# rssalessio/TZDDPC

Measured on AMD Instinct MI355X. Metric: MPC steps/sec (batched trajectories), double-integrator N=20, higher is better.
Workload: dtype f64

## Files before the change

### tzddpc_amd/csrc/tz_ipm.hip.h

```cpp
#pragma once

#define TZ_MINWAVES 4
#define TZ_RLEV_CARRY_MAX 2
#define TZ_RLEV_GATE 1e6
#define TZ_SEED_VIOL_MAX 0.1

struct TzEll { int L, VL; const TzEllEnt* ent; const int* seg; const double* val; const unsigned short* idx; };
#define TZ_ELL_D 8
typedef __attribute__((address_space(1))) const char* tz_gptr;
typedef __attribute__((address_space(1))) const tz_d2* tz_gd2ptr;
#define TZ_ELL_FETCH4(base, r0, r1, r2, r3) \
  tz_d2 r0, r1, r2, r3; \
  { tz_gptr q0 = base, q1 = base + stride, q2 = base + 2 * (size_t)stride, q3 = base + 3 * (size_t)stride; \
    asm volatile("" : "+s"(q0), "+s"(q1), "+s"(q2), "+s"(q3)); \
    r0 = *(tz_gd2ptr)(q0 + lo); r1 = *(tz_gd2ptr)(q1 + lo); r2 = *(tz_gd2ptr)(q2 + lo); r3 = *(tz_gd2ptr)(q3 + lo); \
    base += 4 * (size_t)stride; }
#define TZ_ELL_TERM(r) (r.x * *reinterpret_cast<const double*>(b + tz_ell_off(r.y)))
#define TZ_ELL_APPLY4(a0, a1, r0, r1, r2, r3) { a0 += TZ_ELL_TERM(r0); a1 += TZ_ELL_TERM(r1); a0 += TZ_ELL_TERM(r2); a1 += TZ_ELL_TERM(r3); }
static_assert(TZ_ELL_D == 8, "the windows of tz_ell_walk / tz_ell_walk2 are written out for eight records");
__device__ inline double tz_ell_walk(const char* base_, unsigned lo, int L, unsigned stride, const double* in) {
  double a0 = 0.0, a1 = 0.0;
  const char* b = reinterpret_cast<const char*>(in);
  tz_gptr base = (tz_gptr)base_;
  int e = 0;
// ... 215 lines not shown
  else if (NF == 1) { if (!U0) tz_wave_reduce3<OP0, OP0, OP0, 1>(a, b, c); else if (NV > 1 && !U1) tz_wave_reduce3<OP1, OP1, OP1, 1>(b, a, c); else tz_wave_reduce3<OP2, OP2, OP2, 1>(c, a, b); }
  const int tt = tz_tid();
  int lane = tt & 63, w = tt >> 6;
  double* rb_ = red + (par ? 16 : 0);
  par ^= 1;
  if (lane == 0) {
    rb_[w] = U0 ? __builtin_bit_cast(double, (unsigned long long)ua) : a;
    if (NV > 1) rb_[4 + w] = U1 ? __builtin_bit_cast(double, (unsigned long long)ub) : b;
    if (NV > 2) rb_[8 + w] = U2 ? __builtin_bit_cast(double, (unsigned long long)uc) : c;
  }
  __syncthreads();
  const double ra = tz_fold4<OP0>(rb_), rb = (NV > 1) ? tz_fold4<OP1>(rb_ + 4) : 0.0, rc = (NV > 2) ? tz_fold4<OP2>(rb_ + 8) : 0.0;
  a = ra; if (NV > 1) b = rb; if (NV > 2) c = rc;
}

template <int NCG, int W0 = 0, int NW = TZ_NWAVES>
__device__ inline void tz_gemvT_partial(const double* M, int rows, int nzp, const double* in, double* part) {
  const int tt = tz_tid();
  const int lane = tt & 63, w = (tt >> 6) - W0;
  constexpr int UR = (NCG <= 2) ? 8 : 4;
  double acc[NCG];
#pragma unroll
  for (int g = 0; g < NCG; ++g) acc[g] = 0.0;
  int r = w;
  for (; r + (UR - 1) * NW < rows; r += UR * NW) {
    double v[UR], m[UR][NCG];
#pragma unroll
    for (int u = 0; u < UR; ++u) {
      v[u] = in[r + u * NW];
      const double* row = M + (size_t)(r + u * NW) * nzp;
#pragma unroll
      for (int g = 0; g < NCG; ++g) { const int c = min(lane + 64 * g, nzp - 1); m[u][g] = row[c]; }
    }
#pragma unroll
    for (int u = 0; u < UR; ++u)
#pragma unroll
      for (int g = 0; g < NCG; ++g) acc[g] += m[u][g] * v[u];
  }
  for (; r < rows; r += NW) {
    const double v = in[r];
    const double* row = M + (size_t)r * nzp;
#pragma unroll
    for (int g = 0; g < NCG; ++g) { const int c = min(lane + 64 * g, nzp - 1); acc[g] += row[c] * v; }
  }
#pragma unroll
  for (int g = 0; g < NCG; ++g) { const int c = lane + 64 * g; if (c < nzp) part[w * nzp + c] = acc[g]; }
}
__device__ inline double tz_gemvT_get(const double* part, int nzp, int c) {
  return (part[c] + part[nzp + c]) + (part[2 * nzp + c] + part[3 * nzp + c]);
}
__device__ inline double tz_gemvT_get3(const double* part, int nzp, int c) {
  return (part[c] + part[nzp + c]) + part[2 * nzp + c];
}

template <bool COMPACT>
__device__ inline void tz_ell_gemv_walk(const IpmParams& p, const double* in, double* pl) {
  const int t = tz_tid(), L = p.eg.L;
  int v0 = 0;
  if constexpr (!COMPACT) {
    for (; v0 + TZ_THREADS < p.eg.VL; v0 += 2 * TZ_THREADS) {
      double s0, s1;
      tz_ell_walk2(reinterpret_cast<const char*>(p.eg.ent + (size_t)v0 * L), reinterpret_cast<const char*>(p.eg.ent + (size_t)(v0 + TZ_THREADS) * L),
                   (unsigned)t * 16u, L, TZ_THREADS * 16u, in, s0, s1);
      pl[v0 + t] = s0; pl[v0 + TZ_THREADS + t] = s1;
    }
  }
  for (; v0 < p.eg.VL; v0 += TZ_THREADS) {
    if constexpr (COMPACT) pl[v0 + t] = tz_ell_walk_c(p.eg.val + (size_t)v0 * L + t, p.eg.idx + (size_t)v0 * L + t, L, TZ_THREADS, in);
    else pl[v0 + t] = tz_ell_walk(reinterpret_cast<const char*>(p.eg.ent + (size_t)v0 * L), (unsigned)t * 16u, L, TZ_THREADS * 16u, in);
  }
}
template <int MAXR>
__device__ inline void tz_ell_gemv_sum(const double* pl, const int (&rseg)[MAXR], double (&out)[MAXR]) {
#pragma unroll
  for (int k = 0; k < MAXR; ++k) {
    double a = 0.0;
    int sg = rseg[k];
    asm volatile("" : "+v"(sg));
    const int first = sg & 0xffff, cnt = sg >> 16;
    for (int j = 0; j < cnt; ++j) a += pl[first + j];
    out[k] = a;
  }
}
template <int MAXR, bool COMPACT>
__device__ inline void tz_ell_gemv(const IpmParams& p, const double* in, double* pl, const int (&rseg)[MAXR], double (&out)[MAXR]) {
  __syncthreads();
  tz_ell_gemv_walk<COMPACT>(p, in, pl);
  __syncthreads();
  tz_ell_gemv_sum<MAXR>(pl, rseg, out);
}

template <bool COMPACT>
__device__ inline void tz_ell_gemvT_part(const IpmParams& p, const double* in, double* pl) {
  constexpr int NL = TZ_THREADS - 64;
  const int l = tz_tid() - 64, L = p.et.L;
  for (int v0 = 0; v0 < p.et.VL; v0 += NL) {
    if constexpr (COMPACT) pl[v0 + l] = tz_ell_walk_c(p.et.val + (size_t)v0 * L + l, p.et.idx + (size_t)v0 * L + l, L, NL, in);
    else pl[v0 + l] = tz_ell_walk(reinterpret_cast<const char*>(p.et.ent + (size_t)v0 * L), (unsigned)l * 16u, L, NL * 16u, in);
  }
}
__device__ inline double tz_ell_colsum(const double* pl, int cseg) {
  double a = 0.0;
  asm volatile("" : "+v"(cseg));
  const int first = cseg & 0xffff, cnt = cseg >> 16;
  for (int j = 0; j < cnt; ++j) a += pl[first + j];
  return a;
}

struct TzStage { double a[4]; double b[2]; double w; };

__device__ inline double tz_ld_pinned(const double* p) {
  unsigned long long u = __hip_atomic_load((const unsigned long long*)p, __ATOMIC_RELAXED, __HIP_MEMORY_SCOPE_WAVEFRONT);
  return __builtin_bit_cast(double, u);
}

__device__ inline void tz_form_H(const IpmParams& p, double* Hq, const double* wv, const int* kl) {
  const int lane = threadIdx.x & 63, wave = threadIdx.x >> 6;
  const int k = lane >> 4, blk = (lane >> 2) & 3, ij = lane & 3;
  const int Tz = p.Tz;
  const unsigned rowbytes = (unsigned)(Tz + 1) * 128u;
  const unsigned laneoff = (unsigned)(4 * k + ij) * 8u;
  const char* gp = (const char*)p.Gp;
  const int it0 = __builtin_amdgcn_readfirstlane(p.item_ptr[wave]), it1 = __builtin_amdgcn_readfirstlane(p.item_ptr[wave + 1]);
  for (int it = it0; it < it1; ++it) {
    const IpmItem item = p.items[it];
    const int I0 = __builtin_amdgcn_readfirstlane(item.I0), q0 = __builtin_amdgcn_readfirstlane(item.q0);
    const int nq = __builtin_amdgcn_readfirstlane(item.nq), klen = __builtin_amdgcn_readfirstlane(item.klen);
    const int* kli = kl + __builtin_amdgcn_readfirstlane(item.kptr);
    double acc[4][2];
#pragma unroll
    for (int ii = 0; ii < 4; ++ii) { acc[ii][0] = 0.0; acc[ii][1] = 0.0; }
    unsigned aoff[4], boff[2];
#pragma unroll
    for (int ii = 0; ii < 4; ++ii) aoff[ii] = (unsigned)((I0 + ii < Tz) ? (I0 + ii) : Tz) * 128u + laneoff;
#pragma unroll
    for (int nn = 0; nn < 2; ++nn) { const int J = 4 * (q0 + nn) + blk; boff[nn] = (unsigned)((nn < nq && J < Tz) ? J : Tz) * 128u + laneoff; }
    auto load = [&](int kk, TzStage& st) {
      const int kc = __builtin_amdgcn_readfirstlane(kli[kk]);
      st.w = wv[4 * kc + k];
      const char* prow = gp + (size_t)kc * rowbytes;
#pragma unroll
      for (int ii = 0; ii < 4; ++ii) st.a[ii] = tz_ld_pinned((const double*)(prow + aoff[ii]));
#pragma unroll
      for (int nn = 0; nn < 2; ++nn) st.b[nn] = tz_ld_pinned((const double*)(prow + boff[nn]));
    };
    auto fma8 = [&](const TzStage& st) {
#pragma unroll
      for (int ii = 0; ii < 4; ++ii) {
        const double a = st.a[ii] * st.w;
        acc[ii][0] = __builtin_amdgcn_mfma_f64_4x4x4f64(a, st.b[0], acc[ii][0], 0, 0, 0);
        acc[ii][1] = __builtin_amdgcn_mfma_f64_4x4x4f64(a, st.b[1], acc[ii][1], 0, 0, 0);
      }
    };
    TzStage s0, s1, s2, s3;
    load(0, s0); load(1, s1); load(2, s2);
    for (int kk = 0; kk < klen; kk += 4) {
      load(kk + 3, s3); fma8(s0);
      load(kk + 4, s0); fma8(s1);
      load(kk + 5, s1); fma8(s2);
      load(kk + 6, s2); fma8(s3);
    }
    const int i = lane >> 4, j = lane & 3;
#pragma unroll
    for (int ii = 0; ii < 4; ++ii) {
      const int I = I0 + ii;
      if (I >= Tz) continue;
#pragma unroll
      for (int nn = 0; nn < 2; ++nn) {
        const int q = q0 + nn;
// ... 399 lines not shown
  }
  else for (int i = t; i < p.nklist; i += TZ_THREADS) kl[i] = p.klist[i];
  if (fused) {
    const int n = F0.fin.n, m = F0.fin.m, nv = F0.fin.N * m;
    const int n1 = (F0.tube.pmax + 1) * n * n, n2 = n1 + (F0.tube.pmax > 0 ? F0.tube.pmax : 1) * (n + m) * n;
    for (int i = t; i < n2; i += TZ_THREADS) tbl[i] = (i < n1) ? F0.tube.CKpow[i] : F0.tube.T[i - n1];
    double* ec = tbl + n2;
    const double* plA = F0.plant.A + (size_t)b * F0.plant.A_stride;
    const double* plB = F0.plant.Bm + (size_t)b * F0.plant.B_stride;
    for (int i = t; i < n * n; i += TZ_THREADS) { ec[i] = plA[i]; ec[2 * n * m + n * n + n + i] = F0.fin.R2[i]; ec[2 * n * m + 2 * n * n + n + i] = F0.fin.Phi[(size_t)n * n + i]; }
    for (int i = t; i < n * m; i += TZ_THREADS) { ec[n * n + i] = plB[i]; ec[n * n + n * m + i] = F0.plant.K[i]; }
    for (int i = t; i < n; i += TZ_THREADS) ec[n * n + 2 * n * m + i] = F0.fin.r1[i];
    for (int i = t; i < n * nv; i += TZ_THREADS) ec[3 * n * n + 2 * n * m + n + i] = F0.fin.Gam[(size_t)n * nv + i];
    for (int i = t; i < nv; i += TZ_THREADS) ec[3 * n * n + 2 * n * m + n + n * nv + i] = F0.fin.Dz[i];
    int* pwl = (int*)(ec + 3 * n * n + 2 * n * m + n + n * nv + nv);
    for (int i = t; i < F0.fin.N; i += TZ_THREADS) pwl[i] = F0.tube.power[i];
  }
  if (fused && t < F0.fin.n) {
    stl[t] = F0.plant.x[(size_t)b * F0.fin.n + t];
    stl[F0.fin.n + t] = F0.plant.xbar[(size_t)b * F0.fin.n + t];
    stl[2 * F0.fin.n + t] = F0.plant.e[(size_t)b * F0.fin.n + t];
  }
#pragma unroll
  for (int k = 0; k < MAXR; ++k) { s_[k] = 1.0; l_[k] = 0.0; h_[k] = 0.0; gx_[k] = 0.0; }
  TZ_COLS(c, nzp) xv[c] = 0.0;
  for (int c = t; c < p.Tz * 16; c += TZ_THREADS) dinv[c] = 0.0;
  for (int r = t; r < mip + 4; r += TZ_THREADS) vin[r] = 0.0;
  __syncthreads();

  const int nsteps = fused ? F0.nsteps : 1;
  if (fused && F0.sticky_fresh != 0 && t == 0 && F0.plant.sticky) F0.plant.sticky[b] = 0;
  int was_shifted = (p.warm != 0 && (p.shift_policy >= 2 || p.shift_state[b] == -2)) ? p.shift_state[b] : 0;
  int status = 1, it = 0;
  int work_f = 0, work_s = 0;
  int rlev_carry = 0;
  unsigned brk_hi = 0;
  int rpar = 0;
  for (int step = 0; step < nsteps; ++step) {
  TZ_FRESH_T();
  TzKargPtr kp0 = (TzKargPtr)__builtin_amdgcn_kernarg_segment_ptr();
  asm volatile("" : "+s"(kp0));
  const FuseParams& F = ((const IpmParams*)kp0)->F;
  const IpmParams& pk = *(const IpmParams*)kp0;
  int src = 0;
  if (step == 0) src = (pk.warm != 0 && pk.prev_status != nullptr && pk.prev_status[b] == 0) ? 1 : 0;
  else src = (pk.warm_steps != 0 && status == 0) ? 2 : 0;
  bool skip = false;
  double wpre = 0.0;
  if (fused && t < F.fin.n) wpre = F.plant.w[(size_t)b * F.plant.w_stride + (size_t)step * F.w_step + t];
  bool shifted = false;
  const bool seeded = src != 0 && was_shifted == -2;
  if (seeded) {
    was_shifted = (pk.shift_policy >= 2) ? 1 : 0;
  } else if (src != 0) {
    const int prev_it = (step == 0) ? pk.iters[b] : it;
    const bool quiet_run = was_shifted > 0 && prev_it <= 1;
    const int nquiet = quiet_run ? was_shifted : 0;
    const bool back = was_shifted < 0 && prev_it >= 1;
    shifted = pk.shift_policy == 1 || (pk.shift_policy >= 2 && (prev_it >= pk.shift_policy || back || (quiet_run && (pk.shift_quiet == 0 || nquiet <= pk.shift_quiet))));
    was_shifted = shifted ? 1 + nquiet : (((quiet_run && pk.shift_policy >= 2) || (was_shifted < 0 && !back)) ? -1 : 0);
  }
  const bool inlaunch = fused && src == 2;
  const bool walk_early = inlaunch && (shifted || (step & 7) == 0);
  if (fused) {
    if (t == 0) { flag[0] = 0; flag[1] = 0; }
    const int n = F.fin.n, m = F.fin.m, nv = F.fin.N * m;
    const double* Tt = tbl + (F.tube.pmax + 1) * n * n;
    const int* pwl = (const int*)(Tt + (F.tube.pmax > 0 ? F.tube.pmax : 1) * (n + m) * n + 3 * n * n + 2 * n * m + n + n * nv + nv);
    if (n == 2 && m == 1) tz_tube_stage1<2, 1>(F.tube, tbl, stl + n, stl + 2 * n, Hq, thl, t, TZ_THREADS);
    else tz_tube_stage1(F.tube, tbl, stl + n, stl + 2 * n, Hq, thl, t, TZ_THREADS);
    if (inlaunch && shifted) {
      TZ_COLS(c, nz) tmpz[c] = xv[pk.sx[c]] * pk.sxs[c];
      TZ_ROWS(k, r) vin[r] = l_[k];
    }
    __syncthreads();
    if (n == 2 && m == 1) tz_tube_stage2<2, 1>(F.tube, tbl, Tt, pwl, stl + 2 * n, Hq, thl, t, TZ_THREADS);
    else tz_tube_stage2(F.tube, tbl, Tt, pwl, stl + 2 * n, Hq, thl, t, TZ_THREADS);
    if (inlaunch && shifted) {
      TZ_COLS(c, nz) xv[c] = tmpz[c];
      TZ_ROWS(k, r) l_[k] = vin[pk.sr[r]] * pk.sls[r];
    }
    __syncthreads();
    TZ_STAMP(PH_TUBE);
    TZ_COLS(c, nzp) { qv[c] = (c < nz) ? csr_row(F.qmap, c, thl) : 0.0; if (src != 2) xv[c] = 0.0; }
    TZ_STAMP(PH_MAPS_Q);
    int bad = 0;
    for (int r = t; r < F.npar; r += TZ_THREADS) {
      const double v = csr_row(F.parmap, r, thl);
      if (!(v >= F.par_lo[r] - 1e-9) || !(v <= F.par_hi[r] + 1e-9)) bad = 1;
    }
    if (bad) flag[1] = 1;
    TZ_ROWS(k, r) TZ_SET_H(k, r, csr_row(F.hmap, r, thl));
    if (walk_early) tz_ell_gemv_walk<TT>(p, xv, pl);
  } else {
    TZ_COLS(c, nzp) qv[c] = (c < nz) ? pk.q[(size_t)b * nz + c] : 0.0;
    TZ_ROWS(k, r) TZ_SET_H(k, r, pk.h[(size_t)b * mi + r]);
    if (t == 0) *flag = 0;
  }
  if (src != 2) { TZ_ROWS(k, r) l_[k] = 1.0; }
  if (fused && t < F.fin.n) stl[3 * TZ_NMAX + t] = wpre;
  __syncthreads();
  if (fused && flag[1] != 0) { skip = true; TZ_ROWS(k, r) { s_[k] = 1.0; l_[k] = 0.0; } TZ_COLS(c, nzp) xv[c] = 0.0; }
  TZ_STAMP(PH_PROLOGUE);

  auto exact_rd = [&](bool staged) -> double {
    TZ_STAMP(PH_TEST);
    if (!staged) {
      TZ_ROWS(k, r) vin[r] = l_[k];
      __syncthreads();
    }
    TZ_STAMP(PH_RD_A);
    if (wave0) tz_gemvT_partial<NCG, 0, 1>(p.P, p.nP, nzp, xv, part);
    else tz_ell_gemvT_part<TT>(p, vin, pl);
    __syncthreads();
    TZ_STAMP(PH_RD_B);
    double e1 = 0.0;
    if (nzp <= 64) {
      if (wave0) {
        const double v = (t < nz) ? (tz_ell_colsum(pl, cseg) + qv[t]) + part[t] : 0.0;
        if (t < nzp) rdv[t] = v;
        e1 = tz_wave_reduce<RED_MAX>(fabs(v));
        if (t == 0) red[14] = e1;
      }
      __syncthreads();
      e1 = red[14];
    } else {
      if (t < nzp) rdv[t] = (t < nz) ? (tz_ell_colsum(pl, cseg) + qv[t]) + part[t] : 0.0;
      __syncthreads();
      double e2 = 0, e3 = 0;
      TZ_COLS(c, nz) e1 = fmax(e1, fabs(rdv[c]));
      tz_block_reduce3<RED_MAX, RED_MAX, RED_MAX, 1>(e1, e2, e3, red, rpar);
    }
    TZ_STAMP(PH_RD_C);
    return e1;
  };

  int attempt = 0;
retry_solve:
  const bool retried = attempt != 0;
  bool okf = true;
  bool warm = !skip && src != 0;
  double scq = 0, sch = 0;
  if (!skip) {
  if (warm) {
    if (src == 1) {
      if (shifted) {
        TZ_COLS(c, nz) xv[c] = pk.x[(size_t)b * nz + pk.sx[c]] * pk.sxs[c];
        TZ_ROWS(k, r) l_[k] = pk.lam[(size_t)b * mi + pk.sr[r]] * pk.sls[r];
      } else {
        TZ_COLS(c, nz) xv[c] = pk.x[(size_t)b * nz + c];
        TZ_ROWS(k, r) l_[k] = pk.lam[(size_t)b * mi + r];
      }
    }
    if (walk_early && !retried) { tz_ell_gemv_sum<MAXR>(pl, rseg_, gx_); if (PARK) { TZ_ROWS(k, r) gL[r] = gx_[k]; } }
    else if (src != 2 || retried) { tz_ell_gemv<MAXR, TT>(p, xv, pl, rseg_, gx_); if (PARK) { TZ_ROWS(k, r) gL[r] = gx_[k]; } }
    TZ_STAMP(PH_WARM_A);
    double viol = 0.0;
    TZ_ROWS(k, r) { const double hv = TZ_H(k, r); viol = fmax(viol, TZ_GX(k, r) - hv); sch = fmax(sch, fabs(hv)); }
    TZ_COLS(c, nz) scq = fmax(scq, fabs(qv[c]));
    tz_block_reduce3<RED_MAXU, RED_MAXU, RED_MAXU>(viol, scq, sch, red, rpar);
    TZ_STAMP(PH_WARM_B);
    if (seeded && viol > TZ_SEED_VIOL_MAX) { warm = false; TZ_ROWS(k, r) l_[k] = 1.0; }
    else {
    const double sig = fmin(fmax(pk.warm_floor, pk.warm_gain * viol), pk.warm_cap);
    const double sig2 = sig * sig;
    TZ_ROWS(k, r) {
      s_[k] = fmax(TZ_H(k, r) - TZ_GX(k, r), sig);
      l_[k] = fmax(l_[k], sig2 * tz_recip(s_[k]));
      vin[r] = l_[k];
    }
    }
  }
  if (!warm) {
    was_shifted = 0;
    TZ_ROWS(k, r) vin[r] = 1.0;
// ... 59 lines not shown
      TZ_STAMP(PH_GEMVT);
      if (!(nrd == nrd)) { status = 2; break; }
      if (nrd <= pi.tol_res && nrp <= pi.tol_res && mu <= pi.mu_tol) { status = 0; px_in_part = true; break; }
      if (mu <= pi.mu_floor && !fresh_warm) { status = (nrd <= pi.tol_loose && nrp <= pi.tol_loose) ? 0 : 2; px_in_part = true; break; }
    }
    TZ_ROWS(k, r) { is_[k] = tz_recip(s_[k]); il_[k] = tz_recip(l_[k]); w_[k] = l_[k] * is_[k]; vin[r] = w_[k]; }
    __syncthreads();
    TZ_STAMP(PH_TOP);
    if constexpr (TT) {
      if (rlev == 0 && rlev_carry != 0 && warm && (unsigned)__builtin_amdgcn_readfirstlane((int)tz_hi(mu)) <= brk_hi)
        rlev = rlev_carry < TZ_RLEV_CARRY_MAX ? rlev_carry : TZ_RLEV_CARRY_MAX;
    }
    bool okc;
    __builtin_amdgcn_s_setprio(0);
    if constexpr (TT) tz_gram_tt<TZ_TT_GU(MINW), TZ_TT_NST>(p, Hq, vin, (PROF && t == 0) ? acc_ph : nullptr); else tz_gram(p, Hq, Pq, vin, kl, (PROF && t == 0) ? acc_ph : nullptr);
    __syncthreads();
    TZ_STAMP(PH_FORM);
    TZ_FRESH_T();
    if (rlev != 0) {
      const double rx = (rlev == 1) ? 1e-9 : (rlev == 2) ? 1e-6 : (rlev == 3) ? 1e-3 : 1.0;
      TZ_COLS(c, nz) {
        const int I = c >> 2, i = c & 3;
        Hq[TT ? (size_t)(((I * (I + 1)) >> 1) + I) * p.TS + 5 * i : (size_t)tz_hidx(c, c)] += rx;
      }
    }
    TZ_ROWS(k, r) vin[r] = w_[k] * rp_[k];
    if (t == 0) { flag[2] = 0; flag[3] = 0; }
    __syncthreads();
    if constexpr (!TT) {
      if (wave0) {
        __builtin_amdgcn_s_setprio(TZ_PRIO);
        tz_cholesky_wave(p, Hq, dinv, flag, flag + 2);
        __builtin_amdgcn_s_setprio(0);
      } else {
        tz_ell_gemvT_part<TT>(p, vin, pl);
        tz_gemvT_partial<NCG, 1, 3>(p.P, p.nP, nzp, xv, part2);
        tz_wave_sync();
        if ((tz_tid() & 63) == 0) __hip_atomic_fetch_add(flag + 3, 1, __ATOMIC_RELEASE, __HIP_MEMORY_SCOPE_WORKGROUP);
        if (wave1) {
          bool ok1 = tz_spin_until(flag + 3, 3);
          const int c = tz_tid() & 63;
          double rv = 0.0;
          if (c < nzp) {
            const double pxq = (c < nz) ? tz_gemvT_get3(part2, nzp, c) + qv[c] : 0.0;
            rdv[c] = pxq;
            rv = (c < nz) ? -pxq - tz_ell_colsum(pl, cseg) : 0.0;
          }
          ok1 = tz_fwd_trailing(p, Hq, dinv, rv, flag + 2, tmpz) && ok1;
          if (!ok1 && c == 0) flag[0] = 3;
        }
      }
      __syncthreads();
      okc = (*flag == 0);
      TZ_STAMP(PH_CHOL);
    } else {
      if (wave0) tz_gemvT_partial<NCG, 0, 1>(p.P, p.nP, nzp, xv, part2);
      else tz_ell_gemvT_part<TT>(p, vin, pl);
      __syncthreads();
      TZ_COLS(c, nzp) {
        const double pxq = (c < nz) ? part2[c] + qv[c] : 0.0;
        rdv[c] = pxq;
        r1v[c] = (c < nz) ? -pxq - tz_ell_colsum(pl, cseg) : 0.0;
      }
      __syncthreads();
      TZ_STAMP(PH_GEMVT);
      okc = tz_cholesky_tt(p, Hq, dinv, dfac, flag, (PROF && t == 0) ? acc_ph : nullptr);
      TZ_TT_AFTER_CHOL(p, Hq, dinv);
      TZ_STAMP(PH_CHOL);
    }
    if (!okc) {
      if (rlev >= 4) { status = 2; break; }
      if constexpr (TT) { if (brk_now == 0) brk_now = (unsigned)__builtin_amdgcn_readfirstlane((int)tz_hi(mu * TZ_RLEV_GATE)); }
      rlev = __builtin_amdgcn_readfirstlane(rlev + 1);
      __syncthreads();
      if (t == 0) flag[0] = 0;
      __syncthreads();
      continue;
    }
    TZ_FRESH_T();
    if constexpr (TT) TZ_TT_SOLVE(p, Hq, dinv, r1v, tmpz, dxv);
    else tz_chol_solve_wave(p, Hq, dinv, tmpz, dxv, true);
    __syncthreads();
    TZ_STAMP(PH_SOLVE);
    tz_ell_gemv<MAXR, TT>(p, dxv, pl, rseg_, g_);
    TZ_STAMP(PH_GEMV);
    __builtin_amdgcn_s_setprio(TZ_PRIO_ELEM);
    TZ_FRESH_T();
    double mp = 0.0, md = 0.0, z4 = 0;
    TZ_ROWS(k, r) {
      const double ds = -rp_[k] - g_[k];
      const double dl = -l_[k] - w_[k] * ds;
      ds_[k] = ds; dl_[k] = dl;
      mp = fmax(mp, -ds * is_[k]);
      md = fmax(md, -dl * il_[k]);
      z4 += (s_[k] + ds) * (l_[k] + dl);
    }
    tz_block_reduce3<RED_MAXU, RED_MAXU, RED_SUM>(mp, md, z4, red, rpar);
    const double ap = tz_recip(fmax(1.0, mp)), ad = tz_recip(fmax(1.0, md));
    double muaff = z4;
    if (mp > 1.0 || md > 1.0) {
      double z1 = 0, z2 = 0;
      muaff = 0.0;
      TZ_ROWS(k, r) muaff += (s_[k] + ap * ds_[k]) * (l_[k] + ad * dl_[k]);
      tz_block_reduce3<RED_SUM, RED_SUM, RED_SUM, 1>(muaff, z1, z2, red, rpar);
    }
    muaff *= pi.inv_mi;
    const double sfr = (attempt == 0) ? pi.step_frac : pi.step_frac_retry;
    if (fmin(ap, ad) >= pi.aff_thr && muaff <= pi.aff_mu * mu) {
      const double mmA = fmax(mp, md);
      const double alphaA = (mmA > sfr) ? sfr * tz_recip(mmA) : 1.0;
      TZ_COLS(c, nz) xv[c] += alphaA * dxv[c];
      TZ_ROWS(k, r) { s_[k] += alphaA * ds_[k]; l_[k] += alphaA * dl_[k]; TZ_ADD_GX(k, r, alphaA * g_[k]); }
      __syncthreads();
      continue;
    }
    double sigma = muaff * tz_recip(mu); sigma = sigma * sigma * sigma;
    TZ_FRESH_T();
    TZ_ROWS(k, r) {
      const double rc = s_[k] * l_[k] + ds_[k] * dl_[k] - sigma * mu;
      vin[r] = l_[k] + (l_[k] * rp_[k] - rc) * is_[k];
      ds_[k] = rc;
    }
    __syncthreads();
    TZ_STAMP(PH_ELEM);
    __builtin_amdgcn_s_setprio(0);
    if (!wave0) tz_ell_gemvT_part<TT>(p, vin, pl);
    __syncthreads();
    TZ_COLS(c, nzp) r1v[c] = (c < nz) ? -rdv[c] - tz_ell_colsum(pl, cseg) : 0.0;
    __syncthreads();
    TZ_STAMP(PH_GEMVT);
    if constexpr (TT) TZ_TT_SOLVE(p, Hq, dinv, r1v, tmpz, dxv);
    else tz_chol_solve_wave(p, Hq, dinv, r1v, dxv);
    __syncthreads();
    TZ_STAMP(PH_SOLVE);
    tz_ell_gemv<MAXR, TT>(p, dxv, pl, rseg_, g_);
    TZ_STAMP(PH_GEMV);
    __builtin_amdgcn_s_setprio(TZ_PRIO_ELEM);
    double ms = 0.0, ml = 0.0, z3 = 0;
    TZ_ROWS(k, r) {
      const double rc = ds_[k];
      const double ds = -rp_[k] - g_[k];
      const double dl = (-rc - l_[k] * ds) * is_[k];
      ds_[k] = ds; dl_[k] = dl;
      ms = fmax(ms, -ds * is_[k]);
      ml = fmax(ml, -dl * il_[k]);
    }
    tz_block_reduce3<RED_MAXU, RED_MAXU, RED_SUM, 2>(ms, ml, z3, red, rpar);
    const double mm = fmax(ms, ml);
    const double alpha = (mm * 1.0 > sfr) ? sfr * tz_recip(mm) : 1.0;
    TZ_COLS(c, nz) xv[c] += alpha * dxv[c];
    TZ_ROWS(k, r) { s_[k] += alpha * ds_[k]; l_[k] += alpha * dl_[k]; TZ_ADD_GX(k, r, alpha * g_[k]); }
    __syncthreads();
  }
  __builtin_amdgcn_s_setprio(TZ_PRIO_GLUE);
  TZ_FRESH_T();
  work_f = __builtin_amdgcn_readfirstlane(work_f + it + ((warm || skip) ? 0 : 1));
  if (TT && status == 0 && !skip && attempt == 0) {
    if (brk_now != 0) { rlev_carry = __builtin_amdgcn_readfirstlane(rlev); brk_hi = brk_now; }
    else if (rlev == 0) { rlev_carry = 0; brk_hi = 0; }
  }
  if (status != 0 && !skip && attempt == 0) {
    attempt = 1; src = 0;
    __syncthreads();
    if (t == 0) flag[0] = 0;
    TZ_COLS(c, nzp) xv[c] = 0.0;
    TZ_ROWS(k, r) { s_[k] = 1.0; l_[k] = 1.0; }
    __syncthreads();
    goto retry_solve;
  }
  if (status != 0 && !skip) {
    double lm = 0.0, z1 = 0.0, z2 = 0.0;
    TZ_ROWS(k, r) lm = fmax(lm, l_[k]);
    tz_block_reduce3<RED_MAX, RED_MAX, RED_MAX, 1>(lm, z1, z2, red, rpar);
    const bool lm_ok = lm > 0.0 && lm < 1e300;
    const double il = lm_ok ? 1.0 / lm : 0.0;
    double hy = 0.0;
    TZ_ROWS(k, r) { const double y = lm_ok ? l_[k] * il : 0.0; vin[r] = y; hy += TZ_H(k, r) * y; }
    __syncthreads();
    if (!wave0) tz_ell_gemvT_part<TT>(p, vin, pl);
    __syncthreads();
    double gmax = fabs(tz_ell_colsum(pl, cseg));
    tz_block_reduce3<RED_MAX, RED_SUM, RED_SUM, 2>(gmax, hy, z2, red, rpar);
    if (lm_ok && hy < -1e-6 && gmax <= 1e-6 * fmax(1.0, -hy)) status = 3;
    TZ_COLS(c, nzp) xv[c] = 0.0;
    px_in_part = false;
    __syncthreads();
  }
  work_s += 1;
  TzKargPtr kpe = (TzKargPtr)__builtin_amdgcn_kernarg_segment_ptr();
  asm volatile("" : "+s"(kpe));
  const IpmParams& pe = *(const IpmParams*)kpe;
  if (step == nsteps - 1) {
    TZ_COLS(c, nz) pe.x[(size_t)b * nz + c] = xv[c];
    TZ_ROWS(k, r) { pe.s[(size_t)b * mi + r] = s_[k]; pe.lam[(size_t)b * mi + r] = l_[k]; }
    if (t == 0) {
      pe.status[b] = status; pe.iters[b] = it;
      pe.shift_state[b] = was_shifted;
      if (pe.status_copy) pe.status_copy[b] = status;
      if (pe.work) { atomicAdd(pe.work, (unsigned long long)work_f); atomicAdd(pe.work + 1, (unsigned long long)work_s); atomicMax(pe.work + 2, (unsigned long long)work_f); }
    }
  }
  TZ_STAMP(PH_ELEM);
  if (fused) {
    TzKargPtr kp1 = (TzKargPtr)__builtin_amdgcn_kernarg_segment_ptr();
    asm volatile("" : "+s"(kp1));
    const FuseParams& F = ((const IpmParams*)kp1)->F;
    const int n = F.fin.n, m = F.fin.m, N = F.fin.N, nv = N * m;
    const double* x0 = stl + n;
    const double* ec = tbl + (F.tube.pmax + 1) * n * n + (F.tube.pmax > 0 ? F.tube.pmax : 1) * (n + m) * n;
    const double *cA = ec, *cB = ec + n * n, *cK = cB + n * m, *cr1 = cK + n * m, *cR2 = cr1 + n, *cPhi = cR2 + n * n, *cGam = cPhi + n * n, *cDz = cGam + n * nv;
    const bool want_cost = F.cost_step != 0 || step == nsteps - 1;
    if (F.lean_epilogue != 0 && !want_cost && !F.fin.v && !F.fin.xbar) {
      if (skip) __syncthreads();
      if (t == 0 && status != 0 && F.plant.sticky && F.plant.sticky[b] == 0) F.plant.sticky[b] = status;
      if (t < 64) {
        const PlantParams& Q = F.plant;
        double xn = 0.0, xb = 0.0;
        if (t < n) {
          xn = stl[3 * TZ_NMAX + t];
          for (int j = 0; j < n; ++j) { xn += cA[t * n + j] * stl[j]; xb += cPhi[t * n + j] * x0[j]; }
          for (int j = 0; j < m; ++j) {
            const double v0 = cDz[j] * xv[F.fin.vpos ? F.fin.vpos[j] : j];
            double u = v0;
            for (int i = 0; i < n; ++i) u += cK[j * n + i] * stl[2 * n + i];
            xn += cB[t * m + j] * u; xb += cGam[t * nv + j] * v0;
            if (t == 0 && Q.u_out) Q.u_out[(size_t)b * Q.u_stride + (size_t)step * F.u_step + j] = u;
          }
        }
        __builtin_amdgcn_fence(__ATOMIC_RELEASE, "wavefront");
        __builtin_amdgcn_wave_barrier();
        __builtin_amdgcn_fence(__ATOMIC_ACQUIRE, "wavefront");
        if (t < n) {
          stl[t] = xn; stl[n + t] = xb; stl[2 * n + t] = xn - xb;
          if (Q.x_out) Q.x_out[(size_t)b * Q.x_stride + (size_t)step * F.x_step + t] = xn;
        }
// ... 92 lines not shown
```

### tzddpc_amd/csrc/tz_kernels.hip.h

```cpp
#pragma once
#include <hip/hip_runtime.h>
#include <stdint.h>
#include "tz_layout.h"

#ifndef TZ_PROFILE
#define TZ_PROFILE 0
#endif

typedef double tz_d2 __attribute__((ext_vector_type(2)));
__device__ inline unsigned tz_ell_off(double y) {
  const unsigned long long w = __builtin_bit_cast(unsigned long long, y);
  return (unsigned)w + (unsigned)(w >> 32);
}
struct TzCsr {
  int rows, W;
  const TzEllEnt* ent;
  const double* c0;
};

struct TubeParams {
  int B, n, m, N, pmax, ntheta;
  const double* CKpow;
  const double* T;
  const int* power;
  const double* xbar0; const double* e0;
  double* theta;
  int* prestatus;
};

template <int CTRL>
__device__ inline double tz_quad_xor(double v) {
  const unsigned long long u = __builtin_bit_cast(unsigned long long, v);
  const unsigned lo = (unsigned)__builtin_amdgcn_mov_dpp((int)(unsigned)u, CTRL, 0xf, 0xf, true);
  const unsigned hi = (unsigned)__builtin_amdgcn_mov_dpp((int)(unsigned)(u >> 32), CTRL, 0xf, 0xf, true);
  return __builtin_bit_cast(double, ((unsigned long long)hi << 32) | lo);
}
template <int NC = 0, int MC = 0>
__device__ inline void tz_tube_stage1(const TubeParams& p, const double* CKpow, const double* xbar0, const double* e0, double* aL, double* th, int tid, int nt) {
  const int n = NC ? NC : p.n;
  for (int e = tid; e < p.pmax * n; e += nt) {
    const double* M = CKpow + (size_t)e * n;
    double a = 0.0;
    for (int j = 0; j < n; ++j) a += M[j] * e0[j];
    aL[e] = fabs(a);
  }
  if (tid < n) { const double x0 = xbar0[tid]; th[tid] = x0; th[n + tid] = fabs(x0); }
}
template <int NC = 0, int MC = 0>
__device__ inline void tz_tube_stage2(const TubeParams& p, const double* CKpow, const double* Ttab, const int* power, const double* e0, const double* aL, double* th, int tid, int nt) {
  const int n = NC ? NC : p.n, m = MC ? MC : p.m, hs = 2 * n + m;
  for (int e = tid; e < p.N * n; e += nt) {
    const int k = e / n, i = e - k * n;
    const double* M = CKpow + ((size_t)power[k] * n + i) * n;
    double a = 0.0;
    for (int j = 0; j < n; ++j) a += M[j] * e0[j];
    th[2 * n + k * hs + i] = a;
  }
  const int sub = tid & 3;
  for (int q = tid >> 2; q < p.N * (n + m); q += nt >> 2) {
    const int k = q / (n + m), comp = q - k * (n + m), pw = power[k];
    double a = 0.0;
    for (int l = sub; l < pw; l += 4) {
      const double* T = Ttab + ((size_t)(pw - 1 - l) * (n + m) + comp) * n;
      const double* al = aL + l * n;
      for (int j = 0; j < n; ++j) a += T[j] * al[j];
    }
    a += tz_quad_xor<0xB1>(a);
    a += tz_quad_xor<0x4E>(a);
    if (sub == 0) th[2 * n + k * hs + n + comp] = a;
  }
}
template <int NC = 0, int MC = 0>
__device__ inline void tz_tube_block(const TubeParams& p, const double* CKpow, const double* Ttab, const int* power, const double* xbar0, const double* e0, double* aL, double* th, int tid, int nt) {
  tz_tube_stage1<NC, MC>(p, CKpow, xbar0, e0, aL, th, tid, nt);
  __syncthreads();
  tz_tube_stage2<NC, MC>(p, CKpow, Ttab, power, e0, aL, th, tid, nt);
}

__global__ __launch_bounds__(64) void tz_tube_kernel(TubeParams p) {
  __shared__ double aL[TZ_PMAX * TZ_NMAX];
  const int b = blockIdx.x;
  tz_tube_block(p, p.CKpow, p.T, p.power, p.xbar0 + (size_t)b * p.n, p.e0 + (size_t)b * p.n, aL, p.theta + (size_t)b * p.ntheta, threadIdx.x, 64);
  if (threadIdx.x == 0) p.prestatus[b] = 0;
}

struct AffineParams {
  int B, ntheta, nz, mi, npar;
  TzCsr q, h, par;
  const double* par_lo; const double* par_hi;
  const double* theta;
  double* qv; double* hv;
  int* prestatus;
};

#define TZ_ELL_REG 8
__device__ inline double csr_row(const TzCsr& M, int r, const double* th) {
  double acc = M.c0[r];
  const char* tb = reinterpret_cast<const char*>(th);
  tz_d2 v[TZ_ELL_REG];
#pragma unroll
  for (int e = 0; e < TZ_ELL_REG; ++e) { v[e] = tz_d2{0.0, 0.0}; if (e < M.W) v[e] = *reinterpret_cast<const tz_d2*>(M.ent + (size_t)e * M.rows + r); }
#pragma unroll
  for (int e = 0; e < TZ_ELL_REG; ++e) if (e < M.W) acc += v[e].x * *reinterpret_cast<const double*>(tb + tz_ell_off(v[e].y));
  for (int e = TZ_ELL_REG; e < M.W; ++e) {
    const tz_d2 q = *reinterpret_cast<const tz_d2*>(M.ent + (size_t)e * M.rows + r);
    acc += q.x * *reinterpret_cast<const double*>(tb + tz_ell_off(q.y));
  }
  return acc;
}

__global__ void tz_affine_kernel(AffineParams p) {
  const int rows = p.nz + p.mi + p.npar;
  size_t gid = (size_t)blockIdx.x * blockDim.x + threadIdx.x;
  if (gid >= (size_t)p.B * rows) return;
  int b = (int)(gid / rows), r = (int)(gid % rows);
  const double* th = p.theta + (size_t)b * p.ntheta;
  if (r < p.nz) {
    p.qv[(size_t)b * p.nz + r] = csr_row(p.q, r, th);
  } else if (r < p.nz + p.mi) {
    int rr = r - p.nz;
    p.hv[(size_t)b * p.mi + rr] = csr_row(p.h, rr, th);
  } else {
    int rr = r - p.nz - p.mi;
    double v = csr_row(p.par, rr, th);
    const double tolp = 1e-9;
    if (!(v >= p.par_lo[rr] - tolp) || !(v <= p.par_hi[rr] + tolp)) p.prestatus[b] = 1;
  }
}

struct FinishParams {
  int B, n, m, N, nz, mi, nzp, nc_rows;
  const double* P;  const double* Dz; const double* Phi; const double* Gam;
  const double* r1; const double* R2; double r0; double cost_scale;
  const int* row_of; const double* act_scale;
  const double* xbar0; const double* q; const double* x; const double* s; const double* lam;
  const int* status;
  double* v; double* xbar; double* cost; uint8_t* active;
  size_t cost_stride;
  const int* vpos;
  const double* rec0; const double* recx; const double* recy;
};

struct PlantParams {
  int B, n, m, N;
  const double* K; const double* A; const double* Bm;
  size_t A_stride, B_stride;
  const double* v; const double* xbar_pred;
  const double* w;
  size_t w_stride;
  const int* status;
  double* x; double* xbar; double* e;
  double* u_out; size_t u_stride;
  double* x_out; size_t x_stride;
  int* sticky;
};

struct FuseParams {
  int on;
  int lean_epilogue;
  int sticky_fresh;
  int npar, ntheta;
  int nsteps, warm_steps;
  size_t w_step, u_step, x_step, cost_step;
  TubeParams tube;
  TzCsr qmap, hmap, parmap;
  const double* par_lo; const double* par_hi;
  FinishParams fin;
  PlantParams plant;
};

#include "tz_ipm.hip.h"
#include "tz_identify.hip.h"
#include "tz_genstack.hip.h"
#include "tz_gain.hip.h"

__global__ __launch_bounds__(64) void tz_finish_kernel(FinishParams p) {
  const int b = blockIdx.x, lane = threadIdx.x;
  const int nz = p.nz, n = p.n, m = p.m, N = p.N;
  const double* x = p.x + (size_t)b * nz;
// ... 82 lines not shown
```

Baseline: 104.5 million.

## Prefetch narrow affine-map rows up front and drop redundant IPM barriers

Adds a fixed-width fetch/apply path for ELL maps of width four or less. The q, h and parameter map rows are loaded together before the theta-dependent products, so their global loads can overlap instead of being issued row by row. It also removes the trailing __syncthreads at the end of each IPM iteration and tells the gemv not to issue its leading barrier, since the solve already synchronizes. This relies on no cross-thread hazard existing between the iterate update and the next Cholesky/solve, which is risky if some shared state is read before the next barrier.

```diff
diff --git a/tzddpc_amd/csrc/tz_ipm.hip.h b/tzddpc_amd/csrc/tz_ipm.hip.h
--- a/tzddpc_amd/csrc/tz_ipm.hip.h
+++ b/tzddpc_amd/csrc/tz_ipm.hip.h
@@ -321,9 +321,9 @@
     out[k] = a;
   }
 }
-template <int MAXR, bool COMPACT>
+template <int MAXR, bool COMPACT, bool SYNCED = false>
 __device__ inline void tz_ell_gemv(const IpmParams& p, const double* in, double* pl, const int (&rseg)[MAXR], double (&out)[MAXR]) {
-  __syncthreads();
+  if (!SYNCED) __syncthreads();
   tz_ell_gemv_walk<COMPACT>(p, in, pl);
   __syncthreads();
   tz_ell_gemv_sum<MAXR>(pl, rseg, out);
@@ -889,15 +889,30 @@
     }
     __syncthreads();
     TZ_STAMP(PH_TUBE);
-    TZ_COLS(c, nzp) { qv[c] = (c < nz) ? csr_row(F.qmap, c, thl) : 0.0; if (src != 2) xv[c] = 0.0; }
-    TZ_STAMP(PH_MAPS_Q);
-    int bad = 0;
-    for (int r = t; r < F.npar; r += TZ_THREADS) {
-      const double v = csr_row(F.parmap, r, thl);
-      if (!(v >= F.par_lo[r] - 1e-9) || !(v <= F.par_hi[r] + 1e-9)) bad = 1;
-    }
-    if (bad) flag[1] = 1;
-    TZ_ROWS(k, r) TZ_SET_H(k, r, csr_row(F.hmap, r, thl));
+    if (F.qmap.W <= TZ_MAP_W4 && F.hmap.W <= TZ_MAP_W4 && F.parmap.W <= TZ_MAP_W4 && F.npar <= TZ_THREADS) {
+      const int tw = __builtin_amdgcn_readfirstlane(t) & ~63;
+      const TzMapRow4 Rh = csr_fetch4(F.hmap, min(t, mi - 1));
+      TzMapRow4 Rq = Rh, Rp = Rh; double plo = 0.0, phi = 0.0;
+      if (tw < nz) Rq = csr_fetch4(F.qmap, min(t, nz - 1));
+      if (tw < F.npar) { const int rp = min(t, F.npar - 1); Rp = csr_fetch4(F.parmap, rp); plo = F.par_lo[rp]; phi = F.par_hi[rp]; }
+      TZ_COLS(c, nzp) { qv[c] = (c < nz) ? csr_apply4(F.qmap, Rq, thl) : 0.0; if (src != 2) xv[c] = 0.0; }
+      TZ_STAMP(PH_MAPS_Q);
+      if (t < F.npar) {
+        const double v = csr_apply4(F.parmap, Rp, thl);
+        if (!(v >= plo - 1e-9) || !(v <= phi + 1e-9)) flag[1] = 1;
+      }
+      TZ_ROWS(k, r) TZ_SET_H(k, r, (k == 0) ? csr_apply4(F.hmap, Rh, thl) : csr_row(F.hmap, r, thl));
+    } else {
+      TZ_COLS(c, nzp) { qv[c] = (c < nz) ? csr_row(F.qmap, c, thl) : 0.0; if (src != 2) xv[c] = 0.0; }
+      TZ_STAMP(PH_MAPS_Q);
+      int bad = 0;
+      for (int r = t; r < F.npar; r += TZ_THREADS) {
+        const double v = csr_row(F.parmap, r, thl);
+        if (!(v >= F.par_lo[r] - 1e-9) || !(v <= F.par_hi[r] + 1e-9)) bad = 1;
+      }
+      if (bad) flag[1] = 1;
+      TZ_ROWS(k, r) TZ_SET_H(k, r, csr_row(F.hmap, r, thl));
+    }
     if (walk_early) tz_ell_gemv_walk<TT>(p, xv, pl);
   } else {
     TZ_COLS(c, nzp) qv[c] = (c < nz) ? pk.q[(size_t)b * nz + c] : 0.0;
@@ -1123,7 +1138,7 @@
     else tz_chol_solve_wave(p, Hq, dinv, tmpz, dxv, true);
     __syncthreads();
     TZ_STAMP(PH_SOLVE);
-    tz_ell_gemv<MAXR, TT>(p, dxv, pl, rseg_, g_);
+    tz_ell_gemv<MAXR, TT, true>(p, dxv, pl, rseg_, g_);
     TZ_STAMP(PH_GEMV);
     __builtin_amdgcn_s_setprio(TZ_PRIO_ELEM);
     TZ_FRESH_T();
@@ -1152,7 +1167,6 @@
       const double alphaA = (mmA > sfr) ? sfr * tz_recip(mmA) : 1.0;
       TZ_COLS(c, nz) xv[c] += alphaA * dxv[c];
       TZ_ROWS(k, r) { s_[k] += alphaA * ds_[k]; l_[k] += alphaA * dl_[k]; TZ_ADD_GX(k, r, alphaA * g_[k]); }
-      __syncthreads();
       continue;
     }
     double sigma = muaff * tz_recip(mu); sigma = sigma * sigma * sigma;
@@ -1174,7 +1188,7 @@
     else tz_chol_solve_wave(p, Hq, dinv, r1v, dxv);
     __syncthreads();
     TZ_STAMP(PH_SOLVE);
-    tz_ell_gemv<MAXR, TT>(p, dxv, pl, rseg_, g_);
+    tz_ell_gemv<MAXR, TT, true>(p, dxv, pl, rseg_, g_);
     TZ_STAMP(PH_GEMV);
     __builtin_amdgcn_s_setprio(TZ_PRIO_ELEM);
     double ms = 0.0, ml = 0.0, z3 = 0;
@@ -1191,7 +1205,6 @@
     const double alpha = (mm * 1.0 > sfr) ? sfr * tz_recip(mm) : 1.0;
     TZ_COLS(c, nz) xv[c] += alpha * dxv[c];
     TZ_ROWS(k, r) { s_[k] += alpha * ds_[k]; l_[k] += alpha * dl_[k]; TZ_ADD_GX(k, r, alpha * g_[k]); }
-    __syncthreads();
   }
   __builtin_amdgcn_s_setprio(TZ_PRIO_GLUE);
   TZ_FRESH_T();
diff --git a/tzddpc_amd/csrc/tz_kernels.hip.h b/tzddpc_amd/csrc/tz_kernels.hip.h
--- a/tzddpc_amd/csrc/tz_kernels.hip.h
+++ b/tzddpc_amd/csrc/tz_kernels.hip.h
@@ -94,7 +94,33 @@
 };
 
 #define TZ_ELL_REG 8
+#define TZ_MAP_W4 4
+struct TzMapRow4 { double c0; tz_d2 v0, v1, v2, v3; };
+__device__ inline TzMapRow4 csr_fetch4(const TzCsr& M, int r) {
+  const int W = M.W;
+  const TzEllEnt* b = M.ent + r;
+  const size_t rows = (size_t)M.rows, e1 = (W > 1) ? rows : 0, e2 = (W > 2) ? 2 * rows : e1, e3 = (W > 3) ? 3 * rows : e2;
+  TzMapRow4 R;
+  R.c0 = M.c0[r];
+  R.v0 = *reinterpret_cast<const tz_d2*>(b);
+  R.v1 = *reinterpret_cast<const tz_d2*>(b + e1);
+  R.v2 = *reinterpret_cast<const tz_d2*>(b + e2);
+  R.v3 = *reinterpret_cast<const tz_d2*>(b + e3);
+  return R;
+}
+__device__ inline double csr_apply4(const TzCsr& M, const TzMapRow4& R, const double* th) {
+  const int W = M.W;
+  const char* tb = reinterpret_cast<const char*>(th);
+#define TZ_MAP_TERM(v) (v.x * *reinterpret_cast<const double*>(tb + tz_ell_off(v.y)))
+  double acc = R.c0 + TZ_MAP_TERM(R.v0);
+  const double a1 = acc + TZ_MAP_TERM(R.v1); acc = (W > 1) ? a1 : acc;
+  const double a2 = acc + TZ_MAP_TERM(R.v2); acc = (W > 2) ? a2 : acc;
+  const double a3 = acc + TZ_MAP_TERM(R.v3); acc = (W > 3) ? a3 : acc;
+#undef TZ_MAP_TERM
+  return acc;
+}
 __device__ inline double csr_row(const TzCsr& M, int r, const double* th) {
+  if (M.W <= TZ_MAP_W4) return csr_apply4(M, csr_fetch4(M, r), th);
   double acc = M.c0[r];
   const char* tb = reinterpret_cast<const char*>(th);
   tz_d2 v[TZ_ELL_REG];
```

After: 106.8 million (median of 6 runs). 1.02x the previous value.
